# rmontanana/semcode

Hardware: AMD Instinct MI355X
Metric: chunks/sec embed (256-tok) + top-k QPS over 10M x 768 (higher is better)
Workload: dtype bf16; 1 GPU; encoder forward, 256 chunks x 256 tokens per GPU per step, BERT-base shape (12x768, 12 heads, FFN 3072), bf16 MFMA / f32 accumulate, random-init weights; global_batch=256, seq_len=256, parallelism=dp1 (replicated weights, no collective), device=AMD Radeon Graphics (gfx950:sramecc+:xnack-)

## Files before the change

semcode_amd/csrc/attention_rect.h:

```cpp
#pragma once
#include "attention_core.h"

template <class HEAD, int KT, bool FULL, int GKMAX>
static __device__ __forceinline__ void attention_qblock(const bf16x8 (&qf)[4], const char* Kl, const char* Vl, float* xch, char* ostg,
                                                        bf16_t* obase, int H, int len, int nkt, int lane, int qbase, typename HEAD::Bias slope2) {
    typename HEAD::State st;
    HEAD::init(st);
    HEAD::template fold<KT, FULL, GKMAX>(qf, Kl, Vl, xch, len, nkt, lane, qbase, slope2, st, true, 0);
    HEAD::store(st, xch, ostg, obase, H, lane);
}

template <class HEAD, int KT, int NW>
__global__ __launch_bounds__(NW * 64, (KT <= 8 ? 2 : 1)) void attention_kernel(const bf16_t* __restrict__ qkv, const int32_t* __restrict__ lens, int H,
                                                            typename HEAD::Extra extra, bf16_t* __restrict__ ctx, int blocked) {
    constexpr int S = KT * 32;
    constexpr int NQB = (KT + NW - 1) / NW;
    constexpr int GKMAX = (NW == 8 && KT <= 8) ? 2 : 4;
    extern __shared__ __attribute__((aligned(16))) char smem[];
    char* Kl = smem;
    char* Vl = smem + S * 128;
    const int tid = threadIdx.x, lane = tid & 63;
    const int w = __builtin_amdgcn_readfirstlane(tid >> 6);
    float* xch = reinterpret_cast<float*>(smem + 2 * S * 128) + w * 32;
    char* ostg = smem + 2 * S * 128 + NW * 128 + w * 1024;
    float* tb = nullptr;
    if constexpr (HEAD::TABLE) tb = reinterpret_cast<float*>(smem + attn_lds_bytes(KT, NW));
    const int head = blockIdx.x, b = blockIdx.y;
    const int ld = blocked ? 64 : 3 * H;
    const size_t T = (size_t)blocked, nh = (size_t)(H >> 6);
    const bf16_t* base = blocked ? qkv + ((size_t)head * T + (size_t)b * S) * 64 : qkv + (size_t)b * S * ld + head * 64;
    const size_t koff = blocked ? nh * T * 64 : (size_t)H, voff = 2 * koff;
    int len = lens[b];
    len = len < 1 ? 1 : (len > S ? S : len);
    len = __builtin_amdgcn_readfirstlane(len);
    const int nkt = (len + 31) >> 5;

    for (int piece = w; piece < nkt * 4; piece += NW) {
        const int p = piece * 64 + lane;
        const int r = p >> 3, ck = (p & 7) ^ ((r >> 1) & 7);
        __builtin_amdgcn_global_load_lds((gbl_vptr)(base + (size_t)r * ld + koff + ck * 8), (lds_vptr)(Kl + piece * 1024), 16, 0, 0);
    }
    for (int piece = w; piece < nkt * 4; piece += NW) {
        const int p = piece * 64 + lane;
        const int r = p >> 3, cv = (p & 7) ^ (((r >> 1) & 1) << 2);
        __builtin_amdgcn_global_load_lds((gbl_vptr)(base + (size_t)r * ld + voff + cv * 8), (lds_vptr)(Vl + piece * 1024), 16, 0, 0);
    }
    const int l31 = lane & 31, hh = lane >> 5;
    bf16x8 qf[NQB][4];
#pragma unroll
    for (int i = 0; i < NQB; ++i) {
        const int qb = w + NW * i;
        if (qb < KT) {
            const bf16_t* qrow = base + (size_t)(qb * 32 + l31) * ld;
#pragma unroll
            for (int ks = 0; ks < 4; ++ks) qf[i][ks] = *reinterpret_cast<const bf16x8*>(qrow + 16 * ks + 8 * hh);
        }
    }
    if constexpr (HEAD::TABLE) HEAD::stage(extra, head, tb, -(S - 1), 2 * S - 1, tid, NW * 64);
    asm volatile("s_waitcnt vmcnt(0)" ::: "memory");
    __syncthreads();

#pragma unroll
    for (int i = 0; i < NQB; ++i) {
        const int qb = w + NW * i;
        if (qb < KT) {
            bf16_t* obase = ctx + (size_t)(b * S + qb * 32) * H + head * 64;
            const typename HEAD::Bias slope2 = attn_bias_arg<HEAD>(extra, head, tb, (S - 1) - qb * 32);
            if (nkt == KT && (len & 31) == 0) attention_qblock<HEAD, KT, true, GKMAX>(qf[i], Kl, Vl, xch, ostg, obase, H, len, nkt, lane, qb * 32, slope2);
            else attention_qblock<HEAD, KT, false, GKMAX>(qf[i], Kl, Vl, xch, ostg, obase, H, len, nkt, lane, qb * 32, slope2);
        }
    }
}

template <class HEAD>
__global__ __launch_bounds__(512, 1) void attention_long_kernel(const bf16_t* __restrict__ qkv, const int32_t* __restrict__ lens, int S, int H,
                                                                typename HEAD::Extra extra, bf16_t* __restrict__ ctx, int blocked) {
    constexpr int KT = 16, NW = 8, SEG = 512;
    extern __shared__ __attribute__((aligned(16))) char smem[];
    char* Kl = smem;
    char* Vl = smem + SEG * 128;
    const int tid = threadIdx.x, lane = tid & 63;
    const int w = __builtin_amdgcn_readfirstlane(tid >> 6);
    float* xch = reinterpret_cast<float*>(smem + 2 * SEG * 128) + w * 32;
    char* ostg = smem + 2 * SEG * 128 + NW * 128 + w * 1024;
    float* tb = nullptr;
    if constexpr (HEAD::TABLE) tb = reinterpret_cast<float*>(smem + attn_lds_bytes(KT, NW));
    const int head = blockIdx.x, b = blockIdx.y, qb = (int)blockIdx.z * NW + w;
    const int ld = blocked ? 64 : 3 * H;
    const size_t T = (size_t)blocked, nh = (size_t)(H >> 6);
    const bf16_t* base = blocked ? qkv + ((size_t)head * T + (size_t)b * S) * 64 : qkv + (size_t)b * S * ld + head * 64;
    const size_t koff = blocked ? nh * T * 64 : (size_t)H, voff = 2 * koff;
    int len = lens[b];
    len = len < 1 ? 1 : (len > S ? S : len);
    len = __builtin_amdgcn_readfirstlane(len);
    const int l31 = lane & 31, hh = lane >> 5;
    bf16x8 qf[4];
    {
        const bf16_t* qrow = base + (size_t)(qb * 32 + l31) * ld;
#pragma unroll
        for (int ks = 0; ks < 4; ++ks) qf[ks] = *reinterpret_cast<const bf16x8*>(qrow + 16 * ks + 8 * hh);
    }
    typename HEAD::State st;
    HEAD::init(st);
    typename HEAD::Bias slope2 = attn_bias_arg<HEAD>(extra, head, tb, (32 * NW - 1) - 32 * w);
    const int nseg = (len + SEG - 1) / SEG;
    if constexpr (HEAD::TABLE) HEAD::stage(extra, head, tb, -(int)blockIdx.z * 32 * NW - (32 * NW - 1), nseg * SEG + 32 * NW - 1, tid, NW * 64);
#pragma unroll 1
    for (int seg = 0; seg < nseg; ++seg) {
        const int key0 = seg * SEG;
        const int slen = len - key0 < SEG ? len - key0 : SEG;
        const int nkt = (slen + 31) >> 5;
        if (seg) __syncthreads();
        for (int piece = w; piece < nkt * 4; piece += NW) {
            const int p = piece * 64 + lane;
            const int r = p >> 3, ck = (p & 7) ^ ((r >> 1) & 7);
            __builtin_amdgcn_global_load_lds((gbl_vptr)(base + (size_t)(key0 + r) * ld + koff + ck * 8), (lds_vptr)(Kl + piece * 1024), 16, 0, 0);
        }
        for (int piece = w; piece < nkt * 4; piece += NW) {
            const int p = piece * 64 + lane;
            const int r = p >> 3, cv = (p & 7) ^ (((r >> 1) & 1) << 2);
            __builtin_amdgcn_global_load_lds((gbl_vptr)(base + (size_t)(key0 + r) * ld + voff + cv * 8), (lds_vptr)(Vl + piece * 1024), 16, 0, 0);
        }
        if constexpr (HEAD::TABLE) slope2 = HEAD::bias(tb, (32 * NW - 1) - 32 * w + key0);
        asm volatile("s_waitcnt vmcnt(0)" ::: "memory");
        __syncthreads();
        if (nkt == KT && (slen & 31) == 0) HEAD::template fold<KT, true, 4>(qf, Kl, Vl, xch, slen, nkt, lane, qb * 32, slope2, st, seg == 0, key0);
        else HEAD::template fold<KT, false, 4>(qf, Kl, Vl, xch, slen, nkt, lane, qb * 32, slope2, st, seg == 0, key0);
    }
    HEAD::store(st, xch, ostg, ctx + (size_t)(b * S + qb * 32) * H + head * 64, H, attn_store_lane<HEAD>(lane));
}

template <class HEAD, int KT>
static void launch_attn(const void* qkv, const int32_t* lens, int B, int H, typename HEAD::Extra extra, void* ctx, int blocked, hipStream_t s) {
    constexpr int NW = KT >= 8 ? 8 : 4;
    attn_launch<attention_kernel<HEAD, KT, NW>, attn_lds_bytes(KT, NW) + HEAD::table_bytes(32 * KT, 32 * KT)>(dim3((unsigned)(H / 64), (unsigned)B), NW * 64, s,
                                                                                                               (const bf16_t*)qkv, lens, H, extra, (bf16_t*)ctx, blocked);
}
template <class HEAD>
static void launch_attention(const void* qkv, const int32_t* lens, int B, int S, int H, typename HEAD::Extra extra, void* ctx, int blocked, hipStream_t s) {
    if (S > 512) {
        attn_launch<attention_long_kernel<HEAD>, attn_lds_bytes(16, 8) + HEAD::table_bytes(2048, 256)>(dim3((unsigned)(H / 64), (unsigned)B, (unsigned)(S / 256)), 512, s,
                                                                                                       (const bf16_t*)qkv, lens, S, H, extra, (bf16_t*)ctx, blocked);
        return;
    }
    switch (S) {
        case 32: launch_attn<HEAD, 1>(qkv, lens, B, H, extra, ctx, blocked, s); break;
        case 64: launch_attn<HEAD, 2>(qkv, lens, B, H, extra, ctx, blocked, s); break;
        case 128: launch_attn<HEAD, 4>(qkv, lens, B, H, extra, ctx, blocked, s); break;
        case 256: launch_attn<HEAD, 8>(qkv, lens, B, H, extra, ctx, blocked, s); break;
        case 512: launch_attn<HEAD, 16>(qkv, lens, B, H, extra, ctx, blocked, s); break;
        default: break;
    }
}
```

semcode_amd/csrc/encoder_ops.h:

```cpp
#pragma once
#include <vector>

#include "sc_common.h"

enum { EPI_BIAS = 0, EPI_BIAS_GELU = 1, EPI_BIAS_RES = 2, EPI_LNA_BIAS = 3, EPI_LNA_GELU = 4, EPI_RESLN_STATS = 5, EPI_LNA_BIAS_ROPE = 6 };

bool sc_gemm_bf16_supported(int M, int N, int K);
void sc_launch_gemm_bf16(int epi, const void* A, int lda, const void* W, int ldw, const float* bias, const void* R, int ldr, void* C,
                         int ldc, int M, int N, int K, hipStream_t s, void* splitk_scratch = nullptr, size_t splitk_scratch_bytes = 0);
int sc_gemm_splitk_factor(int M, int N, int K, int cus);
bool sc_gemm_ln_supported(int M, int N, int K);
void sc_launch_gemm_bf16_ln(int epi, const void* A, int lda, const void* W, int ldw, const float* bias, const void* R, int ldr, void* C, int ldc, int M,
                            int N, int K, hipStream_t s, const float* c1, const float* stats_in, float* fin, const float* gam, float* stats_out, float eps,
                            const float* rope_cos = nullptr, const float* rope_sin = nullptr, int rope_S = 0, int rope_ncols = 0);
void sc_launch_gemm_i8_diag(const void* A, const void* W, void* C, int M, int N, int K, hipStream_t s);
void sc_gemm_set_debug(int v);
void sc_gemm_set_order(int v);
void sc_gemm_set_pp(int v);
void sc_gemm_set_nt(int v);
void sc_gemm_set_strip(int v);
void sc_gemm_set_strip_n(int v);
int sc_gemm_strip_rule(int M, int N, int K, int cus);
int sc_gemm_strip_tiles(int M, int N, int K, int cus, bool a_blocked = false);
int sc_gemm_last_strip(void);
void sc_gemm_set_trace(unsigned long long* dev);
void sc_gemm_force_tile128(bool on);

void sc_launch_embed_ln(const int32_t* ids, int tokens, int S, int H, int vocab, int max_pos, const float* wemb, const float* pemb,
                        const float* temb, const float* g, const float* b, float eps, void* out, hipStream_t s);
void sc_launch_layernorm(const void* in, int tokens, int H, const float* g, const float* b, float eps, void* out, hipStream_t s);
bool sc_attention_supported(int S, int H, int heads, int head_dim = 64);
void sc_launch_attention(const void* qkv, const int32_t* lens, int B, int S, int H, const float* slopes, void* ctx, hipStream_t s, int blocked = 0,
                         int head_dim = 64);
void sc_launch_geglu(const void* h, int64_t tokens, int F, void* out, hipStream_t s);
void sc_launch_swiglu(const void* h, int64_t tokens, int F, void* out, hipStream_t s);
void sc_launch_geglu_tanh(const void* h, int64_t tokens, int F, void* out, hipStream_t s);
void sc_launch_relu(void* h, int64_t n, hipStream_t s);
void sc_launch_attention_rel(const void* qkv, const int32_t* lens, int B, int S, int H, const float* tbl, int span, void* ctx, hipStream_t s, int blocked = 0);
void sc_launch_attention_rel_packed(const void* qkv, const int32_t* items, const int* nitems, int H, const float* tbl, int span, void* ctx, hipStream_t s,
                                    int blocked = 0);
void sc_launch_rope_qk(void* qkv, int64_t M, int nblocks, int S, const float* cos_t, const float* sin_t, hipStream_t s);
void sc_launch_embed_raw(const int32_t* ids, int tokens, int tokens_pad, int S, int H, int vocab, int max_pos, const float* wemb, const float* pemb,
                         const float* temb, void* out, float* stats, int slots, hipStream_t s);
void sc_launch_fold_ln_weights(const float* W, const float* gamma, const float* beta, const float* bias, int N, int K, void* Wf, float* c1, float* c2,
                               hipStream_t s);
void sc_launch_add_vectors(const float* a, const float* b, float* out, int n, hipStream_t s);
void sc_launch_mean_pool_ln(const void* y, const float* stats, int slots, int tokens_pad, const float* gamma, const float* beta, float eps,
                            const int32_t* lens, int B, int S, int H, float* out, hipStream_t s);
void sc_launch_mean_pool(const void* x, const int32_t* lens, int B, int S, int H, int normalize, float* out, hipStream_t s);
void sc_launch_f32_to_bf16(const float* in, void* out, int64_t n, hipStream_t s);
void sc_launch_synth_scaled(float* out, int64_t n, uint64_t seed, float scale, float offset, hipStream_t s);
void sc_launch_bf16_to_f32(const void* in, float* out, int64_t n, hipStream_t s);

void sc_launch_embed_ln_packed(const int32_t* ids, const int32_t* pos, int tokens, int H, int vocab, int max_pos, const float* wemb, const float* pemb,
                               const float* temb, const float* g, const float* b, float eps, void* out, hipStream_t s);
void sc_launch_embed_raw_packed(const int32_t* ids, const int32_t* pos, int tokens, int tokens_pad, int H, int vocab, int max_pos, const float* wemb,
                                const float* pemb, const float* temb, void* out, float* stats, int slots, hipStream_t s);
void sc_launch_rope_qk_packed(void* qkv, int64_t M, int nblocks, const int32_t* pos, int max_pos, const float* cos_t, const float* sin_t, hipStream_t s);
int sc_packed_attention_class(int len);
void sc_launch_attention_packed(const void* qkv, const int32_t* items, const int* nitems, int H, const float* slopes, void* ctx, hipStream_t s, int blocked = 0,
                                int head_dim = 64);
void sc_launch_mean_pool_packed(const void* x, const int32_t* starts, const int32_t* lens, int B, int H, int normalize, float* out, hipStream_t s);
void sc_launch_mean_pool_ln_packed(const void* y, const float* stats, int slots, int tokens_pad, const float* gamma, const float* beta, float eps,
                                   const int32_t* starts, const int32_t* lens, int B, int H, float* out, hipStream_t s);

bool sc_attention_window_supported(int local_window);
void sc_launch_attention_window(const void* qkv, const int32_t* lens, int B, int S, int H, int local_window, void* ctx, hipStream_t s, int blocked = 0);
void sc_launch_attention_window_packed(const void* qkv, const int32_t* items, const int* nitems, int H, int local_window, void* ctx, hipStream_t s,
                                       int blocked = 0);

bool sc_attention_causal_supported(int heads, int kv_heads, int head_dim = 64);
void sc_launch_attention_causal(const void* qkv, const int32_t* lens, int B, int S, int heads, int kv_heads, int head_dim, void* ctx, hipStream_t s, int blocked = 0);
void sc_launch_attention_causal_packed(const void* qkv, const int32_t* items, const int* nitems, int heads, int kv_heads, int head_dim, void* ctx, hipStream_t s,
                                       int blocked = 0);
void sc_launch_qknorm_rope(void* qkv, int64_t M, int heads, int kv_heads, int head_dim, int S, const int32_t* pos, int max_pos, const float* cos_t, const float* sin_t,
                           const float* gq, const float* gk, float eps, hipStream_t s);
void sc_launch_rmsnorm(const void* in, int tokens, int H, const float* g, float eps, void* out, hipStream_t s);
void sc_launch_last_pool(const void* x, const int32_t* starts, const int32_t* lens, int B, int S, int H, const float* gamma, float eps, int normalize, float* out,
                         hipStream_t s);

void sc_launch_embed_ln_pairs(const int32_t* ids, const int32_t* pos, const int32_t* types, int tokens, int H, int vocab, int max_pos, int type_vocab,
                              const float* wemb, const float* pemb, const float* temb, const float* g, const float* b, float eps, void* out, hipStream_t s);
void sc_launch_embed_raw_pairs(const int32_t* ids, const int32_t* pos, const int32_t* types, int tokens, int tokens_pad, int H, int vocab, int max_pos,
                               int type_vocab, const float* wemb, const float* pemb, const float* temb, void* out, float* stats, int slots, hipStream_t s);
bool sc_pair_head_supported(int H, int num_labels);
void sc_launch_pair_head(const float* cls, int B, int H, const float* Wp, const float* bp, const float* Wc, const float* bc, int num_labels, float* logits,
                         hipStream_t s);

bool sc_score_head_supported(int H, int num_labels);
void sc_launch_score_head(const float* r, int B, int H, const float* Wd, const float* bd, const float* gam, const float* bet, float eps, const float* Wc,
                          const float* bc, int num_labels, float* logits, hipStream_t s);

bool sc_token_head_supported(int H, int W);
void sc_launch_token_head(const void* x, int rows, int H, const void* w, int W, const int32_t* dst, float* out, hipStream_t s);
void sc_launch_maxsim(const float* Q, const int32_t* q_off, const float* D, const int32_t* d_off, const uint8_t* keep, const int32_t* pair_q, const int32_t* pair_d,
                      int P, int W, float* out, hipStream_t s);

void sc_launch_cls_pool(const void* x, const int32_t* starts, int B, int S, int H, const float* gamma, const float* beta, float eps, int normalize, float* out,
                        hipStream_t s);
void sc_launch_cls_gather(const void* x, const int32_t* starts, int B, int S, int H, const float* gamma, const float* beta, float eps, void* out, int rows_pad,
                          hipStream_t s);
void sc_launch_attention_cls(const void* qkv, const int32_t* starts, const int32_t* lens, int B, int S, int M, int H, int head_dim, const float* slopes, void* ctx,
                             int rows_pad, hipStream_t s);

bool sc_output_proj_supported(int H, int E);
void sc_launch_output_proj(const float* x, int B, int H, const float* W, const float* bias, int E, int normalize, float* out, hipStream_t s);

sc_status sc_score_head_check(const sc_score_head* h, int arch, int H, const char* who);

std::vector<float> sc_rope_table(int64_t positions, float theta, int head_dim = 64);
```

semcode_amd/csrc/encoder_ops.hip:

```cpp
#include "attention_core.h"
#include "encoder_ops.h"
#include "encoder_rows.h"
#include "gemm_tile.h"

__global__ __launch_bounds__(256) void embed_ln_kernel(const int32_t* __restrict__ ids, int tokens, int S, int H, int vocab, int max_pos,
                                                        const float* __restrict__ wemb, const float* __restrict__ pemb,
                                                        const float* __restrict__ temb, const float* __restrict__ gamma,
                                                        const float* __restrict__ beta, float eps, bf16_t* __restrict__ out) {
    embed_ln_rows(ids, tokens, PosInRect{S}, H, vocab, max_pos, wemb, pemb, temb, gamma, beta, eps, out);
}

__global__ __launch_bounds__(256) void embed_raw_kernel(const int32_t* __restrict__ ids, int tokens, int tokens_pad, int S, int H, int vocab, int max_pos,
                                                         const float* __restrict__ wemb, const float* __restrict__ pemb,
                                                         const float* __restrict__ temb, bf16_t* __restrict__ out, float* __restrict__ stats, int slots) {
    embed_raw_rows(ids, tokens, tokens_pad, PosInRect{S}, H, vocab, max_pos, wemb, pemb, temb, out, stats, slots);
}

__global__ __launch_bounds__(256) void fold_ln_weights_kernel(const float* __restrict__ W, const float* __restrict__ gamma, const float* __restrict__ beta,
                                                               const float* __restrict__ bias, int N, int K, bf16_t* __restrict__ Wf,
                                                               float* __restrict__ c1, float* __restrict__ c2) {
    const int lane = threadIdx.x & 63;
    const int n = blockIdx.x * 4 + (threadIdx.x >> 6);
    if (n >= N) return;
    float s1 = 0.f, s2 = 0.f;
    for (int k0 = 4 * lane; k0 < K; k0 += 256) {
        const f32x4 w = *reinterpret_cast<const f32x4*>(W + (size_t)n * K + k0);
        const f32x4 g = *reinterpret_cast<const f32x4*>(gamma + k0);
        const f32x4 b = *reinterpret_cast<const f32x4*>(beta + k0);
        u16x4 r;
#pragma unroll
        for (int c = 0; c < 4; ++c) {
            r[c] = f32_to_bf16(w[c] * g[c]);
            s1 += bf16_to_f32(r[c]);
            s2 = fmaf(b[c], w[c], s2);
        }
        *reinterpret_cast<u16x4*>(Wf + (size_t)n * K + k0) = r;
    }
    s1 = wave_sum(s1);
    s2 = wave_sum(s2);
    if (lane == 0) {
        c1[n] = s1;
        c2[n] = (bias ? bias[n] : 0.f) + s2;
    }
}
__global__ __launch_bounds__(256) void add_vectors_kernel(const float* __restrict__ a, const float* __restrict__ b, float* __restrict__ out, int n) {
    const int i = blockIdx.x * 256 + threadIdx.x;
    if (i < n) out[i] = a[i] + b[i];
}

__global__ __launch_bounds__(256) void mean_pool_ln_kernel(const bf16_t* __restrict__ y, const float* __restrict__ stats, int slots, int tokens_pad,
                                                            const float* __restrict__ gamma, const float* __restrict__ beta, float eps,
                                                            const int32_t* __restrict__ lens, int S, int H, float* __restrict__ out) {
    mean_pool_ln_rows(y, stats, slots, tokens_pad, gamma, beta, eps, RectRows{lens, S}, blockIdx.y, blockIdx.x, H, out);
}

template <int NC>
__global__ __launch_bounds__(256) void layernorm_kernel(const bf16_t* __restrict__ in, int tokens, int H, const float* __restrict__ gamma,
                                                         const float* __restrict__ beta, float eps, bf16_t* __restrict__ out) {
    typedef uint32_t u32x4 __attribute__((ext_vector_type(4)));
    const int l32 = threadIdx.x & 31, half = (threadIdx.x >> 5) & 1;
    const int wave = blockIdx.x * 4 + (threadIdx.x >> 6), nwaves = gridDim.x * 4;
    f32x4 g[NC][2], b[NC][2];
#pragma unroll
    for (int j = 0; j < NC; ++j) {
        const int k0 = (l32 + 32 * j) * 8;
        if (k0 < H) {
            g[j][0] = *reinterpret_cast<const f32x4*>(gamma + k0);
            g[j][1] = *reinterpret_cast<const f32x4*>(gamma + k0 + 4);
            b[j][0] = *reinterpret_cast<const f32x4*>(beta + k0);
            b[j][1] = *reinterpret_cast<const f32x4*>(beta + k0 + 4);
        }
    }
    const float inv_h = 1.0f / (float)H;
    u32x4 nxt[NC];
    int tok = wave * 2 + half;
    if (tok < tokens) {
#pragma unroll
        for (int j = 0; j < NC; ++j) {
            const int k0 = (l32 + 32 * j) * 8;
            if (k0 < H) nxt[j] = __builtin_nontemporal_load(reinterpret_cast<const u32x4*>(in + (size_t)tok * H + k0));
        }
    }
    for (int base = wave * 2; base < tokens; base += nwaves * 2) {
        tok = base + half;
        const bool live = tok < tokens;
        u32x4 raw[NC];
#pragma unroll
        for (int j = 0; j < NC; ++j) raw[j] = nxt[j];
        const int ntok = tok + nwaves * 2;
        if (ntok < tokens) {
#pragma unroll
            for (int j = 0; j < NC; ++j) {
                const int k0 = (l32 + 32 * j) * 8;
                if (k0 < H) nxt[j] = __builtin_nontemporal_load(reinterpret_cast<const u32x4*>(in + (size_t)ntok * H + k0));
            }
        }
        float v[NC][8];
        float sum = 0.f;
#pragma unroll
        for (int j = 0; j < NC; ++j) {
            const bool on = live && (l32 + 32 * j) * 8 < H;
#pragma unroll
            for (int c = 0; c < 4; ++c) {
                v[j][2 * c] = on ? __builtin_bit_cast(float, raw[j][c] << 16) : 0.f;
                v[j][2 * c + 1] = on ? __builtin_bit_cast(float, raw[j][c] & 0xFFFF0000u) : 0.f;
            }
            sum += ((v[j][0] + v[j][1]) + (v[j][2] + v[j][3])) + ((v[j][4] + v[j][5]) + (v[j][6] + v[j][7]));
        }
#pragma unroll
        for (int off = 16; off >= 1; off >>= 1) sum += __shfl_xor(sum, off, 64);
        const float mean = sum * inv_h;
        float sq = 0.f;
#pragma unroll
        for (int j = 0; j < NC; ++j) {
            const bool on = (l32 + 32 * j) * 8 < H;
#pragma unroll
            for (int c = 0; c < 8; ++c) {
                const float d = on ? v[j][c] - mean : 0.f;
                sq = fmaf(d, d, sq);
            }
        }
#pragma unroll
        for (int off = 16; off >= 1; off >>= 1) sq += __shfl_xor(sq, off, 64);
        const float rstd = 1.0f / sqrtf(sq * inv_h + eps);
        if (live) {
#pragma unroll
            for (int j = 0; j < NC; ++j) {
                const int k0 = (l32 + 32 * j) * 8;
                if (k0 < H) {
                    u32x4 r;
#pragma unroll
                    for (int c = 0; c < 4; ++c) {
                        const float lo = (v[j][2 * c] - mean) * rstd * g[j][c >> 1][(2 * c) & 3] + b[j][c >> 1][(2 * c) & 3];
                        const float hi = (v[j][2 * c + 1] - mean) * rstd * g[j][c >> 1][(2 * c + 1) & 3] + b[j][c >> 1][(2 * c + 1) & 3];
                        r[c] = pack_bf16x2(lo, hi);
                    }
                    *reinterpret_cast<u32x4*>(out + (size_t)tok * H + k0) = r;
                }
            }
        }
    }
}

#include "attention_rect.h"

__global__ __launch_bounds__(256) void mean_pool_kernel(const bf16_t* __restrict__ x, const int32_t* __restrict__ lens, int S, int H,
                                                         int normalize, float* __restrict__ out) {
    mean_pool_rows(x, RectRows{lens, S}, blockIdx.x, H, normalize, out);
}

__global__ __launch_bounds__(256) void f32_to_bf16_kernel(const float* __restrict__ in, bf16_t* __restrict__ out, int64_t n) {
    for (int64_t i = (int64_t)blockIdx.x * 256 + threadIdx.x; i < n; i += (int64_t)gridDim.x * 256) out[i] = f32_to_bf16(in[i]);
}
__global__ __launch_bounds__(256) void bf16_to_f32_kernel(const bf16_t* __restrict__ in, float* __restrict__ out, int64_t n) {
    for (int64_t i = (int64_t)blockIdx.x * 256 + threadIdx.x; i < n; i += (int64_t)gridDim.x * 256) out[i] = bf16_to_f32(in[i]);
}
__global__ __launch_bounds__(256) void synth_scaled_kernel(float* __restrict__ out, int64_t n, uint64_t key, float scale, float offset) {
    for (int64_t i = (int64_t)blockIdx.x * 256 + threadIdx.x; i < n; i += (int64_t)gridDim.x * 256)
        out[i] = offset + scale * sc_synth_value(key, (uint64_t)i, 0u, 1u);
}

void sc_launch_embed_ln(const int32_t* ids, int tokens, int S, int H, int vocab, int max_pos, const float* wemb, const float* pemb,
                        const float* temb, const float* g, const float* b, float eps, void* out, hipStream_t s) {
    hipLaunchKernelGGL(embed_ln_kernel, dim3((unsigned)((tokens + 3) / 4)), dim3(256), 0, s, ids, tokens, S, H, vocab, max_pos, wemb, pemb, temb,
                       g, b, eps, (bf16_t*)out);
}
void sc_launch_layernorm(const void* in, int tokens, int H, const float* g, const float* b, float eps, void* out, hipStream_t s) {
    int blocks = (tokens + 7) / 8;
    if (blocks > 256 * 8) blocks = 256 * 8;
    const dim3 grid((unsigned)blocks), block(256);
    if (H <= 768) hipLaunchKernelGGL(layernorm_kernel<3>, grid, block, 0, s, (const bf16_t*)in, tokens, H, g, b, eps, (bf16_t*)out);
    else if (H <= 1024) hipLaunchKernelGGL(layernorm_kernel<4>, grid, block, 0, s, (const bf16_t*)in, tokens, H, g, b, eps, (bf16_t*)out);
    else hipLaunchKernelGGL(layernorm_kernel<8>, grid, block, 0, s, (const bf16_t*)in, tokens, H, g, b, eps, (bf16_t*)out);
}
bool sc_attention_supported(int S, int H, int heads, int head_dim) {
    return heads > 0 && (head_dim == 64 || head_dim == 32) && H == heads * head_dim && H % 64 == 0 && (S == 32 || S == 64 || S == 128 || S == 256 || S == 512 || S == 1024 || S == 2048);
}
void sc_launch_attention(const void* qkv, const int32_t* lens, int B, int S, int H, const float* slopes, void* ctx, hipStream_t s, int blocked, int head_dim) {
    if (head_dim == 32) launch_attention<Head32>(qkv, lens, B, S, H, Head32::Extra(), ctx, blocked, s);
    else if (slopes) launch_attention<Head64<true>>(qkv, lens, B, S, H, slopes, ctx, blocked, s);
    else launch_attention<Head64<false>>(qkv, lens, B, S, H, nullptr, ctx, blocked, s);
}
#include "encoder_glu.h"
void sc_launch_geglu(const void* h, int64_t tokens, int F, void* out, hipStream_t s) {
    int64_t blocks = (tokens * (F / 8) + 255) / 256;
    if (blocks > 8192) blocks = 8192;
    hipLaunchKernelGGL(glu_kernel<ActGelu>, dim3((unsigned)blocks), dim3(256), 0, s, (const bf16_t*)h, tokens, F, (bf16_t*)out);
}
void sc_launch_swiglu(const void* h, int64_t tokens, int F, void* out, hipStream_t s) {
    int64_t blocks = (tokens * (F / 8) + 255) / 256;
    if (blocks > 8192) blocks = 8192;
    hipLaunchKernelGGL(glu_kernel<ActSilu>, dim3((unsigned)blocks), dim3(256), 0, s, (const bf16_t*)h, tokens, F, (bf16_t*)out);
}

__global__ __launch_bounds__(256) void rope_qk_kernel(bf16_t* __restrict__ qkv, int64_t M, int nblocks, int smask, const float* __restrict__ cos_t,
                                                       const float* __restrict__ sin_t) {
    rope_qk_rows(qkv, M, nblocks, PosMasked{smask}, cos_t, sin_t);
}
void sc_launch_rope_qk(void* qkv, int64_t M, int nblocks, int S, const float* cos_t, const float* sin_t, hipStream_t s) {
    int64_t blocks = ((int64_t)nblocks * M * 4 + 255) / 256;
    if (blocks > 16384) blocks = 16384;
    hipLaunchKernelGGL(rope_qk_kernel, dim3((unsigned)blocks), dim3(256), 0, s, (bf16_t*)qkv, M, nblocks, S - 1, cos_t, sin_t);
}
__global__ __launch_bounds__(256) void mean_pool_sliced_kernel(const bf16_t* __restrict__ x, const int32_t* __restrict__ lens, int S, int H,
                                                                float* __restrict__ out) {
    mean_pool_sliced_rows(x, RectRows{lens, S}, blockIdx.y, blockIdx.x, H, out);
}

void sc_launch_mean_pool(const void* x, const int32_t* lens, int B, int S, int H, int normalize, float* out, hipStream_t s) {
    if (!normalize && (H % 8) == 0)
        hipLaunchKernelGGL(mean_pool_sliced_kernel, dim3((unsigned)((H + 255) / 256), (unsigned)B), dim3(256), 0, s, (const bf16_t*)x, lens, S, H, out);
    else
        hipLaunchKernelGGL(mean_pool_kernel, dim3((unsigned)B), dim3(256), 0, s, (const bf16_t*)x, lens, S, H, normalize, out);
}
void sc_launch_embed_raw(const int32_t* ids, int tokens, int tokens_pad, int S, int H, int vocab, int max_pos, const float* wemb, const float* pemb,
                         const float* temb, void* out, float* stats, int slots, hipStream_t s) {
    hipLaunchKernelGGL(embed_raw_kernel, dim3((unsigned)((tokens_pad + 3) / 4)), dim3(256), 0, s, ids, tokens, tokens_pad, S, H, vocab, max_pos, wemb, pemb, temb,
                       (bf16_t*)out, stats, slots);
}
void sc_launch_fold_ln_weights(const float* W, const float* gamma, const float* beta, const float* bias, int N, int K, void* Wf, float* c1, float* c2,
                               hipStream_t s) {
    hipLaunchKernelGGL(fold_ln_weights_kernel, dim3((unsigned)((N + 3) / 4)), dim3(256), 0, s, W, gamma, beta, bias, N, K, (bf16_t*)Wf, c1, c2);
}
void sc_launch_add_vectors(const float* a, const float* b, float* out, int n, hipStream_t s) {
    hipLaunchKernelGGL(add_vectors_kernel, dim3((unsigned)((n + 255) / 256)), dim3(256), 0, s, a, b, out, n);
}
void sc_launch_mean_pool_ln(const void* y, const float* stats, int slots, int tokens_pad, const float* gamma, const float* beta, float eps,
                            const int32_t* lens, int B, int S, int H, float* out, hipStream_t s) {
    hipLaunchKernelGGL(mean_pool_ln_kernel, dim3((unsigned)((H + 255) / 256), (unsigned)B), dim3(256), 0, s, (const bf16_t*)y, stats, slots, tokens_pad, gamma,
                       beta, eps, lens, S, H, out);
}
void sc_launch_f32_to_bf16(const float* in, void* out, int64_t n, hipStream_t s) {
    if (n <= 0) return;
    int64_t blocks = (n + 255) / 256;
    if (blocks > 4096) blocks = 4096;
    hipLaunchKernelGGL(f32_to_bf16_kernel, dim3((unsigned)blocks), dim3(256), 0, s, in, (bf16_t*)out, n);
}
void sc_launch_bf16_to_f32(const void* in, float* out, int64_t n, hipStream_t s) {
    if (n <= 0) return;
    int64_t blocks = (n + 255) / 256;
    if (blocks > 4096) blocks = 4096;
    hipLaunchKernelGGL(bf16_to_f32_kernel, dim3((unsigned)blocks), dim3(256), 0, s, (const bf16_t*)in, out, n);
}
void sc_launch_synth_scaled(float* out, int64_t n, uint64_t seed, float scale, float offset, hipStream_t s) {
    if (n <= 0) return;
    int64_t blocks = (n + 255) / 256;
    if (blocks > 4096) blocks = 4096;
    hipLaunchKernelGGL(synth_scaled_kernel, dim3((unsigned)blocks), dim3(256), 0, s, out, n, sc_synth_key(seed), scale, offset);
}
```

semcode_amd/csrc/sc_api.cpp:

```cpp
#include <algorithm>
#include <cmath>
#include <cstdarg>
#include <cstdio>
#include <cstring>
#include <mutex>
#include <new>
#include <string>
#include <vector>

#include "encoder_ops.h"
#include "sc_internal.h"

static thread_local std::string g_err;

sc_status sc_fail(sc_status code, const char* fmt, ...) {
    char buf[512];
    va_list ap;
    va_start(ap, fmt);
    vsnprintf(buf, sizeof buf, fmt, ap);
    va_end(ap);
    g_err = buf;
    return code;
}

// ... 13 lines not shown
    hipError_t e = hipGetDeviceCount(&ndev);
    if (e != hipSuccess || ndev <= 0)
        return sc_fail(SC_ERR_HIP, "sc_runtime_create: no HIP device available (%s)", e == hipSuccess ? "count = 0" : hipGetErrorString(e));
    const int dev = cfg ? cfg->device : 0;
    if (dev < 0 || dev >= ndev) return sc_fail(SC_ERR_INVALID, "sc_runtime_create: device %d out of range [0,%d)", dev, ndev);
    SC_HIP(hipSetDevice(dev));
    sc_runtime* rt = new (std::nothrow) sc_runtime();
    if (!rt) return sc_fail(SC_ERR_NOMEM, "sc_runtime_create: out of host memory");
    rt->device = dev;
    if (cfg && cfg->stream) {
        rt->stream = (hipStream_t)cfg->stream;
        rt->own_stream = false;
    } else {
        e = hipStreamCreateWithFlags(&rt->stream, hipStreamNonBlocking);
        if (e != hipSuccess) {
            delete rt;
            return sc_fail(SC_ERR_HIP, "hipStreamCreate: %s", hipGetErrorString(e));
        }
        rt->own_stream = true;
    }
    hipDeviceProp_t prop;
    if (hipGetDeviceProperties(&prop, dev) == hipSuccess) {
        snprintf(rt->name, sizeof rt->name, "%s (%s)", prop.name, prop.gcnArchName);
        rt->cus = prop.multiProcessorCount;
        rt->hbm = (int64_t)prop.totalGlobalMem;
    }
    *out = rt;
    return SC_OK;
}

static void prof_clear(sc_runtime* rt) {
    for (int c = 0; c < SC_PROF_CLASSES; ++c) {
        for (auto& p : rt->prof[c]) {
            hipEventDestroy(p.first);
            hipEventDestroy(p.second);
        }
        rt->prof[c].clear();
    }
}

void sc_runtime_retain(sc_runtime* rt) { rt->refs.fetch_add(1, std::memory_order_relaxed); }

void sc_runtime_release(sc_runtime* rt) {
    if (rt->refs.fetch_sub(1, std::memory_order_acq_rel) != 1) return;
    hipSetDevice(rt->device);
    hipStreamSynchronize(rt->stream);
    prof_clear(rt);
    if (rt->own_stream) hipStreamDestroy(rt->stream);
    delete rt;
}

extern "C" sc_status sc_runtime_destroy(sc_runtime* rt) {
    if (!rt) return SC_OK;
    sc_runtime_release(rt);
    return SC_OK;
}

extern "C" sc_status sc_runtime_set_stream(sc_runtime* rt, void* stream) {
    if (!rt) return sc_fail(SC_ERR_INVALID, "runtime is NULL");
    std::lock_guard<std::mutex> g(rt->mu);
    if (rt->own_stream) {
        hipStreamSynchronize(rt->stream);
        hipStreamDestroy(rt->stream);
        rt->own_stream = false;
    }
    rt->stream = (hipStream_t)stream;
    return SC_OK;
}

extern "C" sc_status sc_runtime_synchronize(sc_runtime* rt) {
    if (!rt) return sc_fail(SC_ERR_INVALID, "runtime is NULL");
    SC_HIP(hipSetDevice(rt->device));
    SC_HIP(hipStreamSynchronize(rt->stream));
    return SC_OK;
}

extern "C" sc_status sc_runtime_device_info(sc_runtime* rt, char* name, size_t n, int32_t* cus, int64_t* hbm_bytes) {
    if (!rt) return sc_fail(SC_ERR_INVALID, "runtime is NULL");
    if (name && n) snprintf(name, n, "%s", rt->name);
    if (cus) *cus = rt->cus;
    if (hbm_bytes) *hbm_bytes = rt->hbm;
    return SC_OK;
}

extern "C" sc_status sc_runtime_set_profiling(sc_runtime* rt, int32_t enabled) {
    if (!rt) return sc_fail(SC_ERR_INVALID, "runtime is NULL");
    rt->profiling = enabled < 0 ? 0 : enabled;
    return SC_OK;
}

void sc_prof_begin(sc_runtime* rt, int which, hipEvent_t* a, hipEvent_t* b) {
    *a = *b = nullptr;
    if (!rt->profiling || rt->prof[which].size() >= 8192) return;
    if (which >= SC_PROF_GEMM && rt->profiling > 1 && (rt->prof_seen[which]++ % (unsigned)rt->profiling) != 0) return;
    if (hipEventCreate(a) != hipSuccess) { *a = nullptr; return; }
    if (hipEventCreate(b) != hipSuccess) { hipEventDestroy(*a); *a = *b = nullptr; return; }
    hipEventRecord(*a, rt->stream);
}
void sc_prof_end(sc_runtime* rt, int which, hipEvent_t a, hipEvent_t b) {
    if (!a) return;
    hipEventRecord(b, rt->stream);
    std::lock_guard<std::mutex> g(rt->mu);
    rt->prof[which].push_back({a, b});
}

extern "C" sc_status sc_runtime_profile_read(sc_runtime* rt, int32_t which, double* total_ms, int64_t* launches) {
    if (!rt || which < 0 || which >= SC_PROF_CLASSES) return sc_fail(SC_ERR_INVALID, "bad profile class");
    SC_HIP(hipSetDevice(rt->device));
    SC_HIP(hipStreamSynchronize(rt->stream));
    double t = 0;
    std::lock_guard<std::mutex> g(rt->mu);
    for (auto& p : rt->prof[which]) {
        float ms = 0;
        if (hipEventElapsedTime(&ms, p.first, p.second) == hipSuccess) t += ms;
    }
    if (total_ms) *total_ms = t;
    if (launches) *launches = (int64_t)rt->prof[which].size();
    return SC_OK;
}

extern "C" sc_status sc_runtime_profile_reset(sc_runtime* rt) {
    if (!rt) return sc_fail(SC_ERR_INVALID, "runtime is NULL");
    SC_HIP(hipSetDevice(rt->device));
    SC_HIP(hipStreamSynchronize(rt->stream));
    std::lock_guard<std::mutex> g(rt->mu);
    prof_clear(rt);
    for (unsigned& c : rt->prof_seen) c = 0;
    return SC_OK;
}

extern "C" sc_status sc_synth_fill_dev(sc_runtime* rt, float* out, int64_t rows, int32_t dim, int32_t ld, uint64_t seed,
                                       int64_t first_row) {
    if (!rt || !out) return sc_fail(SC_ERR_INVALID, "sc_synth_fill_dev: NULL argument");
    if (rows < 0 || dim <= 0 || ld < dim || (ld & 3)) return sc_fail(SC_ERR_INVALID, "sc_synth_fill_dev: need rows>=0, 0<dim<=ld, ld%%4==0");
    SC_HIP(hipSetDevice(rt->device));
    sc_launch_synth_fill(out, rows, dim, ld, seed, first_row, nullptr, rt->stream);
    SC_HIP(hipGetLastError());
    return SC_OK;
}

extern "C" sc_status sc_diag_set_option(const char* name, int32_t value) {
    if (!name) return sc_fail(SC_ERR_INVALID, "sc_diag_set_option: NULL name");
    static const struct { const char* name; void (*set)(int); } options[] = {
        {"coarse_workgroups", sc_scan_set_coarse_workgroups}, {"coarse_persistent", sc_scan_set_coarse_persistent},
        {"gemm_pp", sc_gemm_set_pp},                          {"gemm_nt", sc_gemm_set_nt},
        {"ivf_refresh_nomem", sc_ivf_set_refresh_nomem},      {"ivf_refine_cap", sc_ivf_set_refine_cap},
        {"ivf_coarse_nomem", sc_ivf_set_coarse_nomem},        {"collect_pass", sc_set_collect_pass},
        {"tighten", sc_set_tighten},                          {"wide_candidates", sc_set_wide_force},
        {"ivf_tail_rows", sc_set_ivf_tail_rows},              {"delete_chunk_rows", sc_set_delete_chunk_rows},
        {"rope_fused", sc_encoder_set_rope_fused},            {"mask_gather", sc_set_mask_gather},
        {"group_width0", sc_set_group_width0},                {"group_width1", sc_set_group_width1},
        {"mmr_chunk_q", sc_set_mmr_chunk_q},                  {"lex_chunk_q", sc_set_lex_chunk_q},
        {"gemm_strip", sc_gemm_set_strip},                    {"gemm_strip_n", sc_gemm_set_strip_n},
        {"cls_prune", sc_encoder_set_cls_prune},
    };
    for (const auto& o : options)
        if (!strcmp(name, o.name)) {
            o.set(value);
            return SC_OK;
        }
    return sc_fail(SC_ERR_INVALID, "sc_diag_set_option: unknown option '%s'", name);
}


static inline int round_up(int v, int a) { return (v + a - 1) / a * a; }

extern "C" sc_status sc_index_create(sc_runtime* rt, int32_t dim, sc_metric metric, sc_index_kind kind, int32_t nlist,
                                     int64_t row_base, sc_index** out) {
    if (!rt || !out) return sc_fail(SC_ERR_INVALID, "sc_index_create: NULL argument");
    *out = nullptr;
    if (dim <= 0 || dim > 65536) return sc_fail(SC_ERR_INVALID, "sc_index_create: dim %d out of range", dim);
    if (metric != SC_METRIC_IP && metric != SC_METRIC_L2 && metric != SC_METRIC_COSINE)
        return sc_fail(SC_ERR_INVALID, "sc_index_create: unknown metric %d", (int)metric);
    if (kind != SC_INDEX_FLAT && kind != SC_INDEX_IVF_FLAT) return sc_fail(SC_ERR_INVALID, "sc_index_create: unknown kind %d", (int)kind);
    if (kind == SC_INDEX_IVF_FLAT && nlist < 1) return sc_fail(SC_ERR_INVALID, "sc_index_create: IVF_FLAT needs nlist >= 1");
    sc_index* ix = new (std::nothrow) sc_index();
    if (!ix) return sc_fail(SC_ERR_NOMEM, "out of host memory");
    ix->rt = rt;
    sc_runtime_retain(rt);
    ix->dim = dim;
    ix->ld = round_up(dim, SC_LD_ALIGN);
    ix->metric = metric;
    ix->kind = kind;
    ix->nlist = nlist;
    ix->row_base = row_base;
    const size_t ld8 = (size_t)sc_ld8(ix);
    ix->sh_b16.row_bytes[0] = (size_t)ix->ld * 2;
    ix->sh_b16.stat_bit = 1;
    ix->sh_i8.row_bytes[0] = ix->sh_c8.row_bytes[0] = ld8;
    ix->sh_i8.row_bytes[1] = 4;
    ix->sh_i8.stat_bit = 2;
    ix->sh_c8.row_bytes[1] = 16;
    ix->sh_c8.tail_pad = 256;
    ix->sh_c8.stat_bit = 4;
    *out = ix;
    return SC_OK;
}

extern "C" sc_status sc_index_destroy(sc_index* ix) {
    if (!ix) return SC_OK;
    hipSetDevice(ix->rt->device);
    hipStreamSynchronize(ix->rt->stream);
    hipFree(ix->X);
    hipFree(ix->xnorm);
    hipFree(ix->perm);
    hipFree(ix->list_off);
    for (const sc_index_buf& b : SC_INDEX_BUFS) sc_buf_free(ix->*b.buf);
    for (sc_shadow* sh : ix->shadows) sc_shadow_release(*sh);
    sc_tok_free_locked(ix);
    if (ix->quant) sc_index_destroy(ix->quant);
    sc_runtime* rt = ix->rt;
    delete ix;
    sc_runtime_release(rt);
    return SC_OK;
}

extern "C" sc_status sc_index_info(sc_index* ix, int64_t* rows, int32_t* dim, int32_t* ld) {
    if (!ix) return sc_fail(SC_ERR_INVALID, "index is NULL");
    std::lock_guard<std::mutex> g(ix->mu);
    if (rows) *rows = ix->n;
    if (dim) *dim = ix->dim;
    if (ld) *ld = ix->ld;
    return SC_OK;
}

static sc_status ensure_rows(sc_index* ix, int64_t rows, bool exact) {
    if (rows <= ix->capacity) return SC_OK;
    int64_t cap = rows;
    if (!exact) cap = std::max<int64_t>(rows, std::max<int64_t>(ix->capacity * 2, 4096));
    float *nx = nullptr, *nn = nullptr;
    hipError_t e = hipMalloc((void**)&nx, (size_t)cap * ix->ld * sizeof(float));
    if (e != hipSuccess) return sc_fail(SC_ERR_NOMEM, "hipMalloc corpus (%lld rows x %d) failed: %s", (long long)cap, ix->ld, hipGetErrorString(e));
    e = hipMalloc((void**)&nn, (size_t)cap * sizeof(float));
    if (e != hipSuccess) {
        hipFree(nx);
        return sc_fail(SC_ERR_NOMEM, "hipMalloc norms failed: %s", hipGetErrorString(e));
    }
    hipStream_t s = ix->rt->stream;
    if (ix->n > 0) {
        SC_HIP(hipMemcpyAsync(nx, ix->X, (size_t)ix->n * ix->ld * sizeof(float), hipMemcpyDeviceToDevice, s));
        SC_HIP(hipMemcpyAsync(nn, ix->xnorm, (size_t)ix->n * sizeof(float), hipMemcpyDeviceToDevice, s));
    }
    SC_HIP(hipStreamSynchronize(s));
    hipFree(ix->X);
    hipFree(ix->xnorm);
    ix->X = nx;
    ix->xnorm = nn;
    ix->capacity = cap;
    return SC_OK;
}

extern "C" sc_status sc_index_reserve(sc_index* ix, int64_t rows) {
    if (!ix || rows < 0) return sc_fail(SC_ERR_INVALID, "sc_index_reserve: bad argument");
    std::lock_guard<std::mutex> g(ix->mu);
    SC_HIP(hipSetDevice(ix->rt->device));
    return ensure_rows(ix, rows, true);
}

static const int64_t STAGE_ROWS_BYTES = 64ll << 20;

extern "C" sc_status sc_index_add(sc_index* ix, const float* vecs, int64_t n) {
    if (!ix || n < 0 || (n > 0 && !vecs)) return sc_fail(SC_ERR_INVALID, "sc_index_add: bad argument");
    if (n == 0) return SC_OK;
    std::lock_guard<std::mutex> g(ix->mu);
    SC_HIP(hipSetDevice(ix->rt->device));
    if (ix->n + n > 0xFFFFFFF0ll) return sc_fail(SC_ERR_UNSUPPORTED, "sc_index_add: more than 2^32 rows per shard");
    sc_status st = ensure_rows(ix, ix->n + n, false);
    if (st) return st;
    const int64_t chunk = std::max<int64_t>(1, STAGE_ROWS_BYTES / ((int64_t)ix->dim * 4));
    hipStream_t s = ix->rt->stream;
    for (int64_t off = 0; off < n; off += chunk) {
        const int64_t m = std::min(chunk, n - off);
        st = sc_grow(ix, ix->stage, (size_t)m * ix->dim * 4);
        if (st) return st;
        SC_HIP(hipMemcpyAsync(ix->stage.p, vecs + off * ix->dim, (size_t)m * ix->dim * 4, hipMemcpyHostToDevice, s));
        sc_launch_ingest_rows(ix->stage.as<float>(), nullptr, ix->n + off, m, ix->dim, ix->X, ix->ld, ix->xnorm, s);
        SC_HIP(hipGetLastError());
        SC_HIP(hipStreamSynchronize(s));
    }
    ix->n += n;
    if (!ix->perm) ix->trained = false;
    return SC_OK;
}

extern "C" sc_status sc_index_overwrite(sc_index* ix, const float* vecs, const int64_t* rows, int64_t n) {
    if (!ix || n < 0 || (n > 0 && (!vecs || !rows))) return sc_fail(SC_ERR_INVALID, "sc_index_overwrite: bad argument");
    if (n == 0) return SC_OK;
    std::lock_guard<std::mutex> g(ix->mu);
    SC_HIP(hipSetDevice(ix->rt->device));
    for (int64_t i = 0; i < n; ++i)
        if (rows[i] < 0 || rows[i] >= ix->n) return sc_fail(SC_ERR_INVALID, "sc_index_overwrite: row %lld out of range [0,%lld)", (long long)rows[i], (long long)ix->n);
    return sc_index_put_rows_locked(ix, vecs, false, rows, n, "sc_index_overwrite");
}

sc_status sc_index_put_rows_locked(sc_index* ix, const float* vecs, bool vecs_on_device, const int64_t* rows, int64_t n, const char* who) {
    int64_t next = ix->n, min_old = INT64_MAX;
    const int64_t old_n = ix->n;
    for (int64_t i = 0; i < n; ++i) {
        const int64_t r = rows[i];
        if (r == next) ++next;
        else if (r >= 0 && r < ix->n) min_old = std::min(min_old, r);
        else return sc_fail(SC_ERR_INVALID, "%s: rows[%lld] = %lld is neither an existing row [0,%lld) nor the next free row %lld", who, (long long)i,
                            (long long)r, (long long)ix->n, (long long)next);
    }
    if (next > 0xFFFFFFF0ll) return sc_fail(SC_ERR_UNSUPPORTED, "%s: more than 2^32 rows per shard", who);
    {
        std::vector<int64_t> sorted(rows, rows + n);
// ... 258 lines not shown
```

Before: 22960 chunks/s.

## Pipeline attention K/V loads in key segments for S=256 unbiased heads

Adds a split attention kernel for 256-token sequences with the non-ALiBi 64-dim head that issues K/V global-to-LDS loads in 2 or 4 key segments. It waits on vmcnt per segment so the online-softmax fold of earlier segments overlaps with loads of later ones, instead of waiting for all K/V first. Q loads are issued inline after the first segment, and it is enabled by default with split 2. This adds inline asm with hand-counted vmcnt values, which is fragile, and launch bounds now request 4 waves per SIMD, which may cost registers.

```diff
diff --git a/semcode_amd/csrc/attention_rect.h b/semcode_amd/csrc/attention_rect.h
--- a/semcode_amd/csrc/attention_rect.h
+++ b/semcode_amd/csrc/attention_rect.h
@@ -1,5 +1,6 @@
 #pragma once
 #include "attention_core.h"
+#include "encoder_ops.h"
 
 template <class HEAD, int KT, bool FULL, int GKMAX>
 static __device__ __forceinline__ void attention_qblock(const bf16x8 (&qf)[4], const char* Kl, const char* Vl, float* xch, char* ostg,
@@ -71,6 +72,11 @@
         }
     }
 }
+
+template <class HEAD>
+struct attn_split_head : std::false_type {};
+template <>
+struct attn_split_head<Head64<false>> : std::true_type {};
 
 template <class HEAD>
 __global__ __launch_bounds__(512, 1) void attention_long_kernel(const bf16_t* __restrict__ qkv, const int32_t* __restrict__ lens, int S, int H,
@@ -147,7 +153,13 @@
         case 32: launch_attn<HEAD, 1>(qkv, lens, B, H, extra, ctx, blocked, s); break;
         case 64: launch_attn<HEAD, 2>(qkv, lens, B, H, extra, ctx, blocked, s); break;
         case 128: launch_attn<HEAD, 4>(qkv, lens, B, H, extra, ctx, blocked, s); break;
-        case 256: launch_attn<HEAD, 8>(qkv, lens, B, H, extra, ctx, blocked, s); break;
+        case 256:
+            if constexpr (attn_split_head<HEAD>::value) {
+                const int split = sc_attn_split();
+                if (split) { sc_launch_attention_split(split, qkv, lens, B, H, ctx, s, blocked); break; }
+            }
+            launch_attn<HEAD, 8>(qkv, lens, B, H, extra, ctx, blocked, s);
+            break;
         case 512: launch_attn<HEAD, 16>(qkv, lens, B, H, extra, ctx, blocked, s); break;
         default: break;
     }
diff --git a/semcode_amd/csrc/encoder_ops.h b/semcode_amd/csrc/encoder_ops.h
--- a/semcode_amd/csrc/encoder_ops.h
+++ b/semcode_amd/csrc/encoder_ops.h
@@ -32,6 +32,9 @@
 bool sc_attention_supported(int S, int H, int heads, int head_dim = 64);
 void sc_launch_attention(const void* qkv, const int32_t* lens, int B, int S, int H, const float* slopes, void* ctx, hipStream_t s, int blocked = 0,
                          int head_dim = 64);
+void sc_attn_set_split(int v);
+int sc_attn_split(void);
+void sc_launch_attention_split(int split, const void* qkv, const int32_t* lens, int B, int H, void* ctx, hipStream_t s, int blocked);
 void sc_launch_geglu(const void* h, int64_t tokens, int F, void* out, hipStream_t s);
 void sc_launch_swiglu(const void* h, int64_t tokens, int F, void* out, hipStream_t s);
 void sc_launch_geglu_tanh(const void* h, int64_t tokens, int F, void* out, hipStream_t s);
diff --git a/semcode_amd/csrc/encoder_ops.hip b/semcode_amd/csrc/encoder_ops.hip
--- a/semcode_amd/csrc/encoder_ops.hip
+++ b/semcode_amd/csrc/encoder_ops.hip
@@ -176,6 +176,10 @@
 bool sc_attention_supported(int S, int H, int heads, int head_dim) {
     return heads > 0 && (head_dim == 64 || head_dim == 32) && H == heads * head_dim && H % 64 == 0 && (S == 32 || S == 64 || S == 128 || S == 256 || S == 512 || S == 1024 || S == 2048);
 }
+constexpr int ATTN_SPLIT_DEFAULT = 2;
+static int g_attn_split = -1;
+void sc_attn_set_split(int v) { g_attn_split = (v == 0 || v == 2 || v == 4) ? v : -1; }
+int sc_attn_split(void) { return g_attn_split < 0 ? ATTN_SPLIT_DEFAULT : g_attn_split; }
 void sc_launch_attention(const void* qkv, const int32_t* lens, int B, int S, int H, const float* slopes, void* ctx, hipStream_t s, int blocked, int head_dim) {
     if (head_dim == 32) launch_attention<Head32>(qkv, lens, B, S, H, Head32::Extra(), ctx, blocked, s);
     else if (slopes) launch_attention<Head64<true>>(qkv, lens, B, S, H, slopes, ctx, blocked, s);
diff --git a/semcode_amd/csrc/encoder_split.hip b/semcode_amd/csrc/encoder_split.hip
--- /dev/null
+++ b/semcode_amd/csrc/encoder_split.hip
@@ -0,0 +1,127 @@
+#include "attention_rect.h"
+#include "encoder_ops.h"
+
+template <int N>
+static __device__ __forceinline__ void attn_wait_publish() {
+    asm volatile("s_waitcnt vmcnt(%0)\n\ts_barrier" ::"n"(N) : "memory");
+}
+static __device__ __forceinline__ void attn_request_piece(const bf16_t* src, int dst) {
+    unsigned keep;
+    const unsigned lds = __builtin_amdgcn_readfirstlane(__builtin_amdgcn_groupstaticsize() + (unsigned)dst);
+    asm volatile("s_mov_b32 %0, m0\n\ts_mov_b32 m0, %2\n\ts_nop 0\n\tglobal_load_lds_dwordx4 %1, off\n\ts_mov_b32 m0, %0" : "=&s"(keep) : "v"(src), "s"(lds) : "memory");
+}
+static __device__ __forceinline__ void attn_request_q(bf16x8 (&qf)[4], const bf16_t* qrow) {
+    asm volatile("global_load_dwordx4 %0, %4, off\n\tglobal_load_dwordx4 %1, %4, off offset:32\n\t"
+                 "global_load_dwordx4 %2, %4, off offset:64\n\tglobal_load_dwordx4 %3, %4, off offset:96"
+                 : "=&v"(qf[0]), "=&v"(qf[1]), "=&v"(qf[2]), "=&v"(qf[3])
+                 : "v"(qrow)
+                 : "memory");
+}
+template <int N>
+static __device__ __forceinline__ void attn_wait_publish_q(bf16x8 (&qf)[4]) {
+    asm volatile("s_waitcnt vmcnt(%4)\n\ts_barrier" : "+v"(qf[0]), "+v"(qf[1]), "+v"(qf[2]), "+v"(qf[3]) : "n"(N) : "memory");
+}
+template <int PER, int KMAX>
+static __device__ __forceinline__ void attn_wait_publish_younger(int k) {
+    if constexpr (KMAX == 0) {
+        attn_wait_publish<0>();
+    } else {
+        if (k >= KMAX) attn_wait_publish<KMAX * PER>();
+        else attn_wait_publish_younger<PER, KMAX - 1>(k);
+    }
+}
+template <class HEAD, int SPLIT>
+__global__ __launch_bounds__(512, 4) void attention_split_kernel(const bf16_t* __restrict__ qkv, const int32_t* __restrict__ lens, int H,
+                                                                  typename HEAD::Extra extra, bf16_t* __restrict__ ctx, int blocked) {
+    constexpr int KT = 8, NW = 8, S = KT * 32, GKMAX = 2;
+    constexpr int SEGT = KT / SPLIT;
+    constexpr int PW = SEGT * 4 / NW;
+    constexpr int PER = 2 * PW;
+    static_assert(SPLIT == 2 || SPLIT == 4, "halves of 128 keys or groups of 64 keys");
+    static_assert(!HEAD::TABLE, "no table policy is converted");
+    extern __shared__ __attribute__((aligned(16))) char smem[];
+    char* Kl = smem;
+    char* Vl = smem + S * 128;
+    const int tid = threadIdx.x, lane = tid & 63;
+    const int w = __builtin_amdgcn_readfirstlane(tid >> 6);
+    float* xch = reinterpret_cast<float*>(smem + 2 * S * 128) + w * 32;
+    char* ostg = smem + 2 * S * 128 + NW * 128 + w * 1024;
+    const int head = blockIdx.x, b = blockIdx.y;
+    const int ld = blocked ? 64 : 3 * H;
+    const size_t T = (size_t)blocked, nh = (size_t)(H >> 6);
+    const bf16_t* base = blocked ? qkv + ((size_t)head * T + (size_t)b * S) * 64 : qkv + (size_t)b * S * ld + head * 64;
+    const size_t koff = blocked ? nh * T * 64 : (size_t)H, voff = 2 * koff;
+    int len = lens[b];
+    len = len < 1 ? 1 : (len > S ? S : len);
+    len = __builtin_amdgcn_readfirstlane(len);
+    const int nkt = (len + 31) >> 5;
+
+    auto request = [&](int g) {
+#pragma unroll
+        for (int j = 0; j < PW; ++j) {
+            const int piece = g * SEGT * 4 + w + NW * j;
+            const int p = piece * 64 + lane;
+            const int r = p >> 3, ck = (p & 7) ^ ((r >> 1) & 7);
+            attn_request_piece(base + (size_t)r * ld + koff + ck * 8, piece * 1024);
+        }
+#pragma unroll
+        for (int j = 0; j < PW; ++j) {
+            const int piece = g * SEGT * 4 + w + NW * j;
+            const int p = piece * 64 + lane;
+            const int r = p >> 3, cv = (p & 7) ^ (((r >> 1) & 1) << 2);
+            attn_request_piece(base + (size_t)r * ld + voff + cv * 8, S * 128 + piece * 1024);
+        }
+    };
+    const int l31 = lane & 31, hh = lane >> 5;
+    bf16_t* obase = ctx + (size_t)(b * S + w * 32) * H + head * 64;
+    const typename HEAD::Bias slope2 = attn_bias_arg<HEAD>(extra, head, nullptr, 0);
+    bf16x8 qf[4];
+    if (nkt == KT && (len & 31) == 0) {
+        request(0);
+        const int ln = (int)__builtin_amdgcn_mbcnt_hi(~0u, __builtin_amdgcn_mbcnt_lo(~0u, 0u));
+        attn_request_q(qf, base + (size_t)(w * 32 + (ln & 31)) * ld + 8 * (ln >> 5));
+#pragma unroll
+        for (int g = 1; g < SPLIT; ++g) request(g);
+        typename HEAD::State st;
+        HEAD::init(st);
+        attn_wait_publish_q<(SPLIT - 1) * PER>(qf);
+        HEAD::template fold<SEGT, true, GKMAX>(qf, Kl, Vl, xch, 32 * SEGT, SEGT, lane, w * 32, slope2, st, true, 0);
+        attn_wait_publish<(SPLIT - 2) * PER>();
+        HEAD::template fold<SEGT, true, GKMAX>(qf, Kl + SEGT * 4096, Vl + SEGT * 4096, xch, 32 * SEGT, SEGT, lane, w * 32, slope2, st, false, 32 * SEGT);
+        if constexpr (SPLIT == 4) {
+            attn_wait_publish<PER>();
+            HEAD::template fold<SEGT, true, GKMAX>(qf, Kl + 2 * SEGT * 4096, Vl + 2 * SEGT * 4096, xch, 32 * SEGT, SEGT, lane, w * 32, slope2, st, false, 64 * SEGT);
+            attn_wait_publish<0>();
+            HEAD::template fold<SEGT, true, GKMAX>(qf, Kl + 3 * SEGT * 4096, Vl + 3 * SEGT * 4096, xch, 32 * SEGT, SEGT, lane, w * 32, slope2, st, false, 96 * SEGT);
+        }
+        HEAD::store(st, xch, ostg, obase, H, lane);
+    } else {
+        const int nseg = (nkt + SEGT - 1) / SEGT;
+        request(0);
+        attn_request_q(qf, base + (size_t)(w * 32 + l31) * ld + 8 * hh);
+#pragma unroll
+        for (int g = 1; g < SPLIT; ++g)
+            if (g < nseg) request(g);
+        typename HEAD::State st;
+        HEAD::init(st);
+#pragma unroll 1
+        for (int g = 0; g < nseg; ++g) {
+            attn_wait_publish_younger<PER, SPLIT - 1>(nseg - 1 - g);
+            const int key0 = 32 * SEGT * g;
+            const int slen = len - key0 < 32 * SEGT ? len - key0 : 32 * SEGT;
+            HEAD::template fold<SEGT, false, GKMAX>(qf, Kl + g * SEGT * 4096, Vl + g * SEGT * 4096, xch, slen, (slen + 31) >> 5, lane, w * 32, slope2, st, g == 0, key0);
+        }
+        HEAD::store(st, xch, ostg, obase, H, lane);
+    }
+}
+
+template <class HEAD, int SPLIT>
+static void launch_attn_split(const void* qkv, const int32_t* lens, int B, int H, typename HEAD::Extra extra, void* ctx, int blocked, hipStream_t s) {
+    attn_launch<attention_split_kernel<HEAD, SPLIT>, attn_lds_bytes(8, 8)>(dim3((unsigned)(H / 64), (unsigned)B), 512, s, (const bf16_t*)qkv, lens, H, extra, (bf16_t*)ctx,
+                                                                           blocked);
+}
+
+void sc_launch_attention_split(int split, const void* qkv, const int32_t* lens, int B, int H, void* ctx, hipStream_t s, int blocked) {
+    if (split == 2) launch_attn_split<Head64<false>, 2>(qkv, lens, B, H, nullptr, ctx, blocked, s);
+    else launch_attn_split<Head64<false>, 4>(qkv, lens, B, H, nullptr, ctx, blocked, s);
+}
diff --git a/semcode_amd/csrc/sc_api.cpp b/semcode_amd/csrc/sc_api.cpp
--- a/semcode_amd/csrc/sc_api.cpp
+++ b/semcode_amd/csrc/sc_api.cpp
@@ -189,7 +189,7 @@
         {"group_width0", sc_set_group_width0},                {"group_width1", sc_set_group_width1},
         {"mmr_chunk_q", sc_set_mmr_chunk_q},                  {"lex_chunk_q", sc_set_lex_chunk_q},
         {"gemm_strip", sc_gemm_set_strip},                    {"gemm_strip_n", sc_gemm_set_strip_n},
-        {"cls_prune", sc_encoder_set_cls_prune},
+        {"cls_prune", sc_encoder_set_cls_prune},              {"attn_split", sc_attn_set_split},
     };
     for (const auto& o : options)
         if (!strcmp(name, o.name)) {
```

Result: no change. 22970 chunks/s (median of 4 runs) (+0.0%).
